# Tianxinhuang/RFNet

Hardware: AMD Instinct MI355X
Metric: point-pairs/sec Chamfer (BxNxM) (higher is better)
Workload: dtype f32; 1 GPU; Chamfer nn_distance fwd+bwd, B=32 per GPU, 2048 vs 16384 points (BASELINE.json configs[1]), randn seed 100; batch_per_gpu=32, n=2048, m=16384, step=rf_chamfer_step: one C-ABI call, caller-allocated outputs

## Files before the change

### rfnet_amd/csrc/nn_pruned.hip

```cpp
#include <stdlib.h>

#include <type_traits>

#include "common.hpp"
#include "nn_pruned.hpp"

namespace {

#ifndef RFP_NSH
#define RFP_NSH 4
#endif
#ifndef RFP_SPLIT_BELOW
#define RFP_SPLIT_BELOW 4096
#endif
#ifndef RFP_SORT_SPLIT
#define RFP_SORT_SPLIT 2
#endif
#ifndef RFP_SORT_SPLIT_ABOVE
#define RFP_SORT_SPLIT_ABOVE 8192
#endif
#ifndef RFP_WPE
#define RFP_WPE 7
#endif
#ifndef RFP_QSAMPLE
#define RFP_QSAMPLE 3
#endif
#ifndef RFP_STR_SMALL_N
#define RFP_STR_SMALL_N 4096
#endif
#ifndef RFP_CROWD_DIV
#define RFP_CROWD_DIV 4
#endif
#ifndef RFP_STR_LARGE_LEAF
#define RFP_STR_LARGE_LEAF 48
#endif
#ifndef RFP_STR_SMALL_LEAF
#define RFP_STR_SMALL_LEAF 32
#endif
#ifndef RFP_TILE16
#define RFP_TILE16 1
#endif
#ifndef RFP_KK1
#define RFP_KK1 1
#endif
#ifndef RFP_REKEY_BOX
#define RFP_REKEY_BOX 1
#endif
#ifndef RFP_REKEY_STATS
#define RFP_REKEY_STATS 0
#endif
constexpr int NSH = RFP_NSH;
constexpr int BS = 16;
constexpr int SBB = 4;
constexpr int SB = BS * SBB;
constexpr int KEYBITS = 15;
constexpr int NBINS = 1 << KEYBITS;
constexpr int STPB = 1024;
constexpr int RPT = 16;
constexpr int HB = 256;
static_assert(rfp::kMaxPoints / SB <= 1024, "superblock id must fit the key low 10 bits");
static_assert(!RFP_TILE16 || NSH == SBB, "the quad-per-query tiles need one wave per 16-record block of a group: RFP_NSH = 4");
constexpr unsigned IDMASK = 0x3FFu;
constexpr int B16F = SBB * 6;
constexpr int B64F = 8;

struct SortArgs {
    int b;
    int n[2], npad[2];
    const float *src[2];
    float *xyz[2];
    int *orig[2];
    float *box16[2];
    float *box64[2];
    int nsets;
    int split[2];
    int *pos0[2];
    int str_s[2];
    unsigned long long *dbg;
};

__device__ __forceinline__ int ragged_count(const int *__restrict__ len, int bi, int n) {
    if (!len) return n;
    const int v = len[bi];
    return v < 1 ? 1 : (v > n ? n : v);
}

__device__ __forceinline__ unsigned hilbert15(unsigned x, unsigned y, unsigned z) {
    unsigned X[3] = {x, y, z};
#pragma unroll
    for (unsigned Q = 16; Q > 1; Q >>= 1) {
        const unsigned P = Q - 1;
#pragma unroll
        for (int i = 0; i < 3; i++) {
            if (X[i] & Q) {
                X[0] ^= P;
            } else {
                const unsigned t = (X[0] ^ X[i]) & P;
                X[0] ^= t;
                X[i] ^= t;
            }
        }
    }
    X[1] ^= X[0];
    X[2] ^= X[1];
    unsigned t = 0;
#pragma unroll
    for (unsigned Q = 16; Q > 1; Q >>= 1)
        if (X[2] & Q) t ^= Q - 1;
    X[0] ^= t;
    X[1] ^= t;
    X[2] ^= t;
    unsigned key = 0;
#pragma unroll
    for (int bit = 0; bit < 5; bit++)
#pragma unroll
        for (int i = 0; i < 3; i++) key |= ((X[i] >> bit) & 1u) << (3 * bit + 2 - i);
    return key & (NBINS - 1);
}

__device__ __forceinline__ float axis_off(float lo, float scale) {
    return fmaf(-lo, scale, -0.5f);
}
__device__ __forceinline__ int axis_bin(float v, float off, float scale) {
    static_assert(HB == 256, "a bin is a byte");
    return (int)__builtin_amdgcn_cvt_pk_u8_f32(fmaf(v, scale, off), 0, 0u);
}
__device__ __forceinline__ float canon(float v) {
    asm volatile("v_max_f32 %0, %0, %0" : "+v"(v));
    return v;
}
__device__ __forceinline__ float bare_min(float a, float b) {
    float r;
    asm("v_min_f32 %0, %1, %2" : "=v"(r) : "v"(a), "v"(b));
    return r;
}
__device__ __forceinline__ float bare_max(float a, float b) {
    float r;
    asm("v_max_f32 %0, %1, %2" : "=v"(r) : "v"(a), "v"(b));
    return r;
}

__device__ __forceinline__ unsigned spread5(unsigned v) {
    v = (v | (v << 8)) & 0x100Fu;
    v = (v | (v << 4)) & 0x10C3u;
    v = (v | (v << 2)) & 0x1249u;
    return v;
}

__device__ __forceinline__ unsigned wave_incl_scan(unsigned v) {
    v += (unsigned)__builtin_amdgcn_update_dpp(0, (int)v, 0x111, 0xf, 0xf, false);
    v += (unsigned)__builtin_amdgcn_update_dpp(0, (int)v, 0x112, 0xf, 0xf, false);
    v += (unsigned)__builtin_amdgcn_update_dpp(0, (int)v, 0x114, 0xf, 0xf, false);
    v += (unsigned)__builtin_amdgcn_update_dpp(0, (int)v, 0x118, 0xf, 0xf, false);
    v += (unsigned)__builtin_amdgcn_update_dpp(0, (int)v, 0x142, 0xa, 0xf, false);
    v += (unsigned)__builtin_amdgcn_update_dpp(0, (int)v, 0x143, 0xc, 0xf, false);
    return v;
}

#define RFP_ROW(OP, N) asm volatile("s_nop 1\n\t" OP " %0, %0, %0 row_ror:" #N " row_mask:0xf bank_mask:0xf" : "+v"(v))
__device__ __forceinline__ float wave_min_f32(float v) {
    RFP_ROW("v_min_f32_dpp", 8);
    RFP_ROW("v_min_f32_dpp", 4);
    RFP_ROW("v_min_f32_dpp", 2);
    RFP_ROW("v_min_f32_dpp", 1);
    const float r0 = __int_as_float(__builtin_amdgcn_readlane(__float_as_int(v), 0));
    const float r1 = __int_as_float(__builtin_amdgcn_readlane(__float_as_int(v), 16));
    const float r2 = __int_as_float(__builtin_amdgcn_readlane(__float_as_int(v), 32));
    const float r3 = __int_as_float(__builtin_amdgcn_readlane(__float_as_int(v), 48));
    return fminf(fminf(r0, r1), fminf(r2, r3));
}
__device__ __forceinline__ float wave_max_f32(float v) {
    RFP_ROW("v_max_f32_dpp", 8);
    RFP_ROW("v_max_f32_dpp", 4);
    RFP_ROW("v_max_f32_dpp", 2);
    RFP_ROW("v_max_f32_dpp", 1);
    const float r0 = __int_as_float(__builtin_amdgcn_readlane(__float_as_int(v), 0));
    const float r1 = __int_as_float(__builtin_amdgcn_readlane(__float_as_int(v), 16));
    const float r2 = __int_as_float(__builtin_amdgcn_readlane(__float_as_int(v), 32));
    const float r3 = __int_as_float(__builtin_amdgcn_readlane(__float_as_int(v), 48));
    return fmaxf(fmaxf(r0, r1), fmaxf(r2, r3));
}
#undef RFP_ROW

__device__ __forceinline__ bool hist_is_dense(unsigned bin, bool act) {
    const unsigned long long todo = __builtin_amdgcn_ballot_w64(act);
    if (todo == 0ull) return false;
    const unsigned first = (unsigned)__builtin_amdgcn_readlane((int)bin, __builtin_ctzll(todo));
    return __builtin_popcountll(__builtin_amdgcn_ballot_w64(act && bin == first)) >= 8;
}

constexpr int HALF = 9216;

template <bool RAGGED, bool FLAG>
__global__ __launch_bounds__(STPB) void nnp_sort_reg_kernel(SortArgs a, const int *__restrict__ len0,
                                                            const int *__restrict__ len1) {
    struct Lds {
        unsigned ahist[3][HB];
        unsigned char slabmap[HB];
        unsigned short zmap[HB];
        unsigned char stripmap[16 * HB];
        float red[STPB / 64][6];
        unsigned wsum[STPB / 64];
        unsigned lowcnt[STPB / 64][3];
        float frame[6];
        unsigned ncrowded;
        unsigned badw[STPB / 64];
        __attribute__((aligned(16))) unsigned hist[HALF * 4];
    };
    __shared__ Lds lds;
    auto &hist = lds.hist;
    auto &ahist = lds.ahist;
    auto &slabmap = lds.slabmap;
    auto &zmap = lds.zmap;
    auto &stripmap = lds.stripmap;
    auto &red = lds.red;
    auto &wsum = lds.wsum;
    auto &lowcnt = lds.lowcnt;
    auto &frame = lds.frame;
    auto &ncrowded = lds.ncrowded;
    auto &badw = lds.badw;

    const int nwg = gridDim.x, q8 = nwg >> 3, r8 = nwg & 7, xcd = blockIdx.x & 7;
    const int logical = (xcd < r8 ? xcd * (q8 + 1) : r8 * (q8 + 1) + (xcd - r8) * q8) + (int)(blockIdx.x >> 3);
    if (threadIdx.x == 0) ncrowded = 0;
    const int wpb = a.split[0] + (a.nsets > 1 ? a.split[1] : 0);
    const int bi = logical / wpb;
    int rem = logical - bi * wpb;
    const int set = (a.nsets > 1 && rem >= a.split[0]) ? 1 : 0;
    if (set) rem -= a.split[0];
    const int H = a.split[set], half = rem;
    const int nfull = a.n[set], npad = a.npad[set];
    const float *__restrict__ src = a.src[set] + (size_t)bi * nfull * 3;
    const int n = RAGGED ? ragged_count(set ? len1 : len0, bi, nfull) : nfull;
    float *__restrict__ oxyz = a.xyz[set] + (size_t)bi * npad * 3;
    int *__restrict__ oorig = a.orig[set] + (size_t)bi * npad;
    const int tid = threadIdx.x, lane = tid & 63, wave = tid >> 6;
    int stamp_no = 16;
    auto stamp = [&]() {
        if (a.dbg && bi == a.b - 1 && set == a.nsets - 1 && half == H - 1 && tid == 0 && stamp_no < 32) a.dbg[stamp_no] = clock64();
        stamp_no++;
    };
    stamp();

    float px[RPT], py[RPT], pz[RPT];
    unsigned pk[RPT];
#pragma unroll
    for (int k = 0; k < RPT; k++) {
        const int i = tid + k * STPB;
        px[k] = py[k] = pz[k] = 0.f;
        if (i < n) {
            struct P3 {
                float x, y, z;
            };
            const P3 v = *(const P3 *)(src + (size_t)i * 3);
            px[k] = v.x;
            py[k] = v.y;
            pz[k] = v.z;
        }
    }
    {
        uint4 *h4 = (uint4 *)hist;
#pragma unroll
        for (int k = 0; k < NBINS / 4 / STPB; k++) h4[tid + k * STPB] = make_uint4(0, 0, 0, 0);
    }
    if (tid < 3 * HB) (&ahist[0][0])[tid] = 0;
    unsigned *yhist = hist + NBINS;
    for (int i = tid; i < 16 * HB; i += STPB) yhist[i] = 0;

    stamp();
    {
#pragma unroll
        for (int k = 0; k < RPT; k++) {
            px[k] = canon(px[k]);
            py[k] = canon(py[k]);
            pz[k] = canon(pz[k]);
        }
        float lo[3] = {INFINITY, INFINITY, INFINITY}, hi[3] = {-INFINITY, -INFINITY, -INFINITY};
#define RFP_BBOX_PASS(FILTER)                                                     \
    _Pragma("unroll") for (int k = 0; k < RPT; k++) {                             \
        if (tid + k * STPB < n) {                                                 \
            const float v[3] = {px[k], py[k], pz[k]};                             \
            _Pragma("unroll") for (int c = 0; c < 3; c++) {                       \
                if (!(FILTER) || isfinite(v[c])) {                                \
                    lo[c] = bare_min(lo[c], v[c]);                                \
                    hi[c] = bare_max(hi[c], v[c]);                                \
                }                                                                 \
            }                                                                     \
        }                                                                         \
    }                                                                             \
    _Pragma("unroll") for (int c = 0; c < 3; c++) {                               \
        lo[c] = wave_min_f32(lo[c]);                                              \
        hi[c] = wave_max_f32(hi[c]);                                              \
    }
        RFP_BBOX_PASS(false)
        if (!(isfinite(lo[0]) && isfinite(lo[1]) && isfinite(lo[2]) && isfinite(hi[0]) && isfinite(hi[1]) && isfinite(hi[2]))) {
#pragma unroll
            for (int c = 0; c < 3; c++) {
                lo[c] = INFINITY;
                hi[c] = -INFINITY;
            }
            RFP_BBOX_PASS(true)
        }
#undef RFP_BBOX_PASS
        if (lane == 0) {
#pragma unroll
            for (int c = 0; c < 3; c++) {
                red[wave][c] = lo[c];
                red[wave][3 + c] = hi[c];
            }
        }
        if (FLAG) {
            float nf = 0.f;
#pragma unroll
            for (int k = 0; k < RPT; k++) nf = fmaf(pz[k], 0.f, fmaf(py[k], 0.f, fmaf(px[k], 0.f, nf)));
            const unsigned long long bad_lanes = __ballot(nf != nf);
            if (lane == 0) badw[wave] = bad_lanes != 0ull ? 1u : 0u;
        }
    }
    __syncthreads();
    if (tid < 3) {
        float l = INFINITY, h = -INFINITY;
        for (int w = 0; w < STPB / 64; w++) {
            l = bare_min(l, red[w][tid]);
            h = bare_max(h, red[w][3 + tid]);
        }
        const float ext = h - l;
        const bool ok = isfinite(ext) && ext > 0.f;
        frame[tid] = ok ? l : 0.f;
        frame[3 + tid] = ok ? (float)HB / ext : 0.f;
    }
    __syncthreads();
    const float fs[3] = {frame[3], frame[4], frame[5]};
    const float fl[3] = {axis_off(frame[0], fs[0]), axis_off(frame[1], fs[1]), axis_off(frame[2], fs[2])};

    stamp();
    bool dense;
    {
        const int w3 = wave & RFP_QSAMPLE;
        const float x0 = w3 == 0 ? px[0] : (w3 == 3 ? px[1] : (w3 == 2 ? px[2] : px[3]));
        const int k0 = (4 - w3) & 3;
        dense = RFP_QSAMPLE == 3 && hist_is_dense((unsigned)axis_bin(x0, fl[0], fs[0]), tid + k0 * STPB < n);
    }
    const bool feeds = !dense || (lane & 3) == 0;
    if (dense && lane == 0) atomicAdd(&ncrowded, 1u);
#pragma unroll
    for (int k = 0; k < RPT; k++) {
        if (((k + wave) & RFP_QSAMPLE) != 0) continue;
        if (feeds && tid + k * STPB < n) {
            atomicAdd(&ahist[0][axis_bin(px[k], fl[0], fs[0])], 1u);
            atomicAdd(&ahist[2][axis_bin(pz[k], fl[2], fs[2])], 1u);
        }
        __builtin_amdgcn_sched_barrier(0);
    }
    __syncthreads();
    const int SS = a.str_s[set];
    if (wave == 0 || wave == 2) {
        unsigned c4[4], sm = 0;
#pragma unroll
        for (int k = 0; k < 4; k++) {
            c4[k] = ahist[wave][lane * 4 + k];
            sm += c4[k];
        }
        const unsigned incl = wave_incl_scan(sm);
        const unsigned total = max((unsigned)__builtin_amdgcn_readlane((int)incl, 63), 1u);
        unsigned run = incl - sm;
        const float per = (wave == 0 ? (float)SS : 512.f) / (float)total;
#pragma unroll
        for (int k = 0; k < 4; k++) {
            const unsigned q = (unsigned)((float)run * per);
            if (wave == 0) {
                slabmap[lane * 4 + k] = (unsigned char)(q > (unsigned)SS - 1u ? (unsigned)SS - 1u : q);
            } else {
                zmap[lane * 4 + k] = (unsigned short)(q > 511u ? 511u : q);
            }
            run += c4[k];
        }
    }
    __syncthreads();
#pragma unroll
    for (int k = 0; k < RPT; k++) {
        if (((k + wave) & RFP_QSAMPLE) != 0) continue;
        if (feeds && tid + k * STPB < n)
            atomicAdd(&yhist[(int)slabmap[axis_bin(px[k], fl[0], fs[0])] * HB + axis_bin(py[k], fl[1], fs[1])], 1u);
    }
    __syncthreads();
    if (wave < SS) {
        unsigned c4[4], sm = 0;
#pragma unroll
        for (int k = 0; k < 4; k++) {
            c4[k] = yhist[wave * HB + lane * 4 + k];
            sm += c4[k];
        }
        const unsigned incl = wave_incl_scan(sm);
        const unsigned total = max((unsigned)__builtin_amdgcn_readlane((int)incl, 63), 1u);
        unsigned run = incl - sm;
        const float per = (float)SS / (float)total;
#pragma unroll
        for (int k = 0; k < 4; k++) {
            unsigned st = (unsigned)((float)run * per);
            st = st > (unsigned)SS - 1u ? (unsigned)SS - 1u : st;
            stripmap[wave * HB + lane * 4 + k] = (unsigned char)((wave & 1) ? (unsigned)SS - 1u - st : st);
            run += c4[k];
        }
    }
    __syncthreads();
    const int ncol = SS * SS;
    auto col_start = [&](int q) { return (q * ncol + H - 1) / H; };
    const int cs1 = H > 1 ? col_start(1) : 0x7FFFFFFF;
#if RFP_SORT_SPLIT > 2
    const int cs2 = H > 2 ? col_start(2) : 0x7FFFFFFF, cs3 = H > 3 ? col_start(3) : 0x7FFFFFFF;
#endif
    const unsigned kbase = (unsigned)col_start(half) << 9;
    const int nb_local = (col_start(half + 1) - col_start(half)) << 9;

    stamp();
    unsigned below[3] = {0u, 0u, 0u};
    const unsigned dkeep = dense ? ~15u : ~0u, dlane = dense ? (unsigned)(lane & 15) : 0u;
#pragma unroll
    for (int k = 0; k < RPT; k++) {
        const bool valid = tid + k * STPB < n;
        const int xb = axis_bin(px[k], fl[0], fs[0]), yb = axis_bin(py[k], fl[1], fs[1]);
        const int slab = slabmap[xb];
        const int col = (int)__umul24(slab, SS) + (int)stripmap[slab * HB + yb];
#if RFP_SORT_SPLIT > 2
        int slice = col >= cs1;
        if (H > 2) slice += (col >= cs2) + (col >= cs3);
        const bool own = valid && slice == half;
#pragma unroll
        for (int q = 0; q < 3; q++) below[q] += (unsigned)__builtin_popcountll(__builtin_amdgcn_ballot_w64(valid && slice == q));
#else
        const bool own = valid && (col >= cs1) == (half != 0);
#endif
        unsigned zq = zmap[axis_bin(pz[k], fl[2], fs[2])];
        zq = (zq & dkeep) | dlane;
        const unsigned key = ((unsigned)col << 9) | ((col & 1) ? 511u - zq : zq);
        pk[k] = own ? key - kbase : 0xFFFFFFFFu;
        if (own) atomicAdd(&hist[pk[k]], 1u);
    }
#if RFP_SORT_SPLIT <= 2
    if (half == 1) {
#pragma unroll
        for (int k = 0; k < RPT; k++) {
            const int nv = n - (__builtin_amdgcn_readfirstlane(wave) * 64 + k * STPB);
            below[0] += (unsigned)(nv < 0 ? 0 : (nv > 64 ? 64 : nv)) - (unsigned)__builtin_popcountll(__builtin_amdgcn_ballot_w64(pk[k] != 0xFFFFFFFFu));
        }
    }
#endif
    if (H > 1 && lane == 0) {
#pragma unroll
        for (int q = 0; q < 3; q++) lowcnt[wave][q] = q < half ? below[q] : 0u;
    }
    __syncthreads();

    stamp();
    int cown = 0;
    {
        constexpr int STEPS = NBINS / (STPB / 64) / 256;
        const int steps = min(STEPS, (nb_local + 4095) / 4096);
        uint4 *h4 = (uint4 *)hist + (size_t)wave * steps * 64;
        uint4 v[STEPS];
        unsigned tot = 0;
#pragma unroll
        for (int it = 0; it < STEPS; it++) {
            v[it] = it < steps ? h4[it * 64 + lane] : make_uint4(0, 0, 0, 0);
            tot += v[it].x + v[it].y + v[it].z + v[it].w;
        }
        tot = wave_incl_scan(tot);
        if (lane == 63) wsum[wave] = tot;
        __syncthreads();
        const unsigned wtot = lane < STPB / 64 ? wsum[lane] : 0u;
        const unsigned wincl = wave_incl_scan(wtot);
        unsigned carry = (unsigned)__builtin_amdgcn_readlane((int)(wincl - wtot), __builtin_amdgcn_readfirstlane(wave));
        cown = __builtin_amdgcn_readlane((int)wincl, STPB / 64 - 1);
#pragma unroll
        for (int it = 0; it < STEPS; it++) {
            if (it < steps) {
                const unsigned sm = v[it].x + v[it].y + v[it].z + v[it].w;
                const unsigned incl = wave_incl_scan(sm);
                uint4 out;
                out.x = carry + incl - sm;
                out.y = out.x + v[it].x;
                out.z = out.y + v[it].y;
                out.w = out.z + v[it].z;
                h4[it * 64 + lane] = out;
                carry += (unsigned)__builtin_amdgcn_readlane((int)incl, 63);
            }
        }
    }
    __syncthreads();

    stamp();
#pragma unroll
    for (int k = 0; k < RPT; k++)
        if (pk[k] != 0xFFFFFFFFu) pk[k] = atomicAdd(&hist[pk[k]], 1u);
    __syncthreads();

    stamp();
    float4 *stg = (float4 *)hist;
    float *__restrict__ b16 = a.box16[set] + (size_t)bi * (npad / SB) * B16F;
    float *__restrict__ b64 = a.box64[set] + (size_t)bi * (npad / SB) * B64F;
    int base = 0;
    for (int q = 0; q < half; q++) {
        unsigned c = 0;
        for (int w = 0; w < STPB / 64; w++) c += lowcnt[w][q];
        base += ((int)c + SB - 1) / SB * SB;
    }
    const int seglen = ((cown + SB - 1) / SB) * SB;
    if (half == H - 1) {
        const int t0 = base + seglen;
        for (int j = t0 * 3 + tid; j < npad * 3; j += STPB) oxyz[j] = INFINITY;
        for (int j = t0 + tid; j < npad; j += STPB) oorig[j] = -1;
        for (int j = (t0 / SB) * B16F + tid; j < (npad / SB) * B16F; j += STPB) b16[j] = ((j % 6) < 3) ? INFINITY : -INFINITY;
        for (int j = (t0 / SB) * B64F + tid; j < (npad / SB) * B64F; j += STPB) {
            const int c = j % B64F;
            b64[j] = c < 3 ? INFINITY : (c >= 4 && c < 7 ? -INFINITY : 0.f);
        }
    }
    if (tid == 0 && pk[0] != 0xFFFFFFFFu) a.pos0[set][bi] = base + (int)pk[0];
    if (tid == 0 && half == 0) {
        a.pos0[set][a.b + bi] = ncrowded * RFP_CROWD_DIV > STPB / 64 ? 1 : 0;
        if (FLAG) {
            unsigned nbad = 0;
            for (int w = 0; w < STPB / 64; w++) nbad |= badw[w];
            a.pos0[set][2 * a.b + bi] = nbad != 0u ? 1 : 0;
        }
    }
    for (int h0 = 0; h0 < seglen; h0 += HALF) {
        const int cnt = min(HALF, seglen - h0);
#pragma unroll
        for (int k = 0; k < RPT; k++) {
            const int i = tid + k * STPB;
            const int p = (int)pk[k] - h0;
            if (pk[k] != 0xFFFFFFFFu && p >= 0 && p < HALF) stg[p] = make_float4(px[k], py[k], pz[k], __int_as_float(i));
        }
        for (int p = cown - h0 + tid; p < cnt; p += STPB)
            if (p >= 0) stg[p] = make_float4(INFINITY, INFINITY, INFINITY, __int_as_float(-1));
        __syncthreads();
        stamp();
#pragma unroll 1
        for (int t2 = tid; t2 < cnt / BS * 2; t2 += STPB) {
            const int blk = t2 >> 1, hf = t2 & 1;
            float l[3] = {INFINITY, INFINITY, INFINITY}, hh[3] = {-INFINITY, -INFINITY, -INFINITY};
#pragma unroll 4
            for (int u = 0; u < BS / 2; u++) {
                const int r = blk * BS + hf * (BS / 2) + ((u + blk + 4 * hf) & (BS / 2 - 1));
                const float4 v = stg[r];
                if (h0 + r < cown) {
                    l[0] = bare_min(l[0], v.x); hh[0] = bare_max(hh[0], v.x);
                    l[1] = bare_min(l[1], v.y); hh[1] = bare_max(hh[1], v.y);
                    l[2] = bare_min(l[2], v.z); hh[2] = bare_max(hh[2], v.z);
                }
            }
#pragma unroll
            for (int c = 0; c < 3; c++) {
                l[c] = bare_min(l[c], __shfl_xor(l[c], 1, 64));
                hh[c] = bare_max(hh[c], __shfl_xor(hh[c], 1, 64));
            }
            const int gblk = (base + h0) / BS + blk;
            if (hf == 0) {
                float *o = b16 + (size_t)(gblk >> 2) * B16F + (gblk & 3) * 6;
#pragma unroll
                for (int c = 0; c < 3; c++) {
                    o[c] = l[c];
                    o[3 + c] = hh[c];
                }
            }
#pragma unroll
            for (int x = 2; x <= 4; x <<= 1) {
#pragma unroll
                for (int c = 0; c < 3; c++) {
                    l[c] = bare_min(l[c], __shfl_xor(l[c], x, 64));
                    hh[c] = bare_max(hh[c], __shfl_xor(hh[c], x, 64));
                }
            }
            if ((gblk & 3) == 0 && hf == 0) {
                float *o64 = b64 + (size_t)(gblk >> 2) * B64F;
#pragma unroll
                for (int c = 0; c < 3; c++) {
                    o64[c] = l[c];
                    o64[4 + c] = hh[c];
                }
                o64[3] = o64[7] = 0.f;
            }
        }
        stamp();
        {
            struct P3 {
                float x, y, z;
            };
            for (int j = tid; j < cnt; j += STPB) {
                const float4 v = stg[j];
                *(P3 *)(oxyz + (size_t)(base + h0 + j) * 3) = P3{v.x, v.y, v.z};
                oorig[base + h0 + j] = __float_as_int(v.w);
            }
        }
        __syncthreads();
        stamp();
    }
}

template <bool REG, bool RAGGED>
__global__ __launch_bounds__(STPB) void nnp_sort_kernel(SortArgs a, const int *__restrict__ len0,
                                                        const int *__restrict__ len1) {
    __shared__ __attribute__((aligned(16))) unsigned hist[NBINS];
    __shared__ unsigned ahist[3][HB];
    __shared__ unsigned char cellmap[3][HB];
    __shared__ float red[STPB / 64][6];
    __shared__ unsigned wsum[STPB / 64];
    __shared__ float frame[6];
    __shared__ unsigned nbad;

    const int nwg = gridDim.x, q8 = nwg >> 3, r8 = nwg & 7, xcd = blockIdx.x & 7;
    const int logical = (xcd < r8 ? xcd * (q8 + 1) : r8 * (q8 + 1) + (xcd - r8) * q8) + (int)(blockIdx.x >> 3);
    const int bi = logical / a.nsets, set = logical - bi * a.nsets;
    if (threadIdx.x == 0) nbad = 0;
    const int nfull = a.n[set], npad = a.npad[set];
    const float *__restrict__ src = a.src[set] + (size_t)bi * nfull * 3;
    const int n = RAGGED ? ragged_count(set ? len1 : len0, bi, nfull) : nfull;
    float *__restrict__ oxyz = a.xyz[set] + (size_t)bi * npad * 3;
    int *__restrict__ oorig = a.orig[set] + (size_t)bi * npad;
    const int tid = threadIdx.x, lane = tid & 63, wave = tid >> 6;

    float px[REG ? RPT : 1], py[REG ? RPT : 1], pz[REG ? RPT : 1];
    unsigned pkey[REG ? RPT : 1];
    if constexpr (REG) {
#pragma unroll
        for (int k = 0; k < RPT; k++) {
            const int i = tid + k * STPB;
            px[k] = py[k] = pz[k] = 0.f;
            if (i < n) {
                px[k] = src[(size_t)i * 3 + 0];
                py[k] = src[(size_t)i * 3 + 1];
                pz[k] = src[(size_t)i * 3 + 2];
            }
        }
    }
    auto for_points = [&](auto f) {
        if constexpr (REG) {
#pragma unroll
            for (int k = 0; k < RPT; k++) {
                const int i = tid + k * STPB;
                if (i < n) f(k, i, px[k], py[k], pz[k]);
            }
        } else {
            for (int i = tid; i < n; i += STPB) f(0, i, src[(size_t)i * 3 + 0], src[(size_t)i * 3 + 1], src[(size_t)i * 3 + 2]);
        }
    };

    for (int i = tid; i < NBINS; i += STPB) hist[i] = 0;
    if (tid < 3 * HB) (&ahist[0][0])[tid] = 0;

    float lo[3] = {INFINITY, INFINITY, INFINITY}, hi[3] = {-INFINITY, -INFINITY, -INFINITY};
    bool bad = false;
    __syncthreads();
    for_points([&](int, int, float x, float y, float z) {
        const float v[3] = {x, y, z};
#pragma unroll
        for (int c = 0; c < 3; c++) {
            if (isfinite(v[c])) {
                lo[c] = fminf(lo[c], v[c]);
                hi[c] = fmaxf(hi[c], v[c]);
            } else {
                bad = true;
            }
        }
    });
    if (__ballot(bad) != 0ull && lane == 0) nbad = 1u;
#pragma unroll
    for (int o = 32; o > 0; o >>= 1) {
#pragma unroll
        for (int c = 0; c < 3; c++) {
            lo[c] = fminf(lo[c], __shfl_xor(lo[c], o, 64));
            hi[c] = fmaxf(hi[c], __shfl_xor(hi[c], o, 64));
        }
    }
    if (lane == 0) {
#pragma unroll
        for (int c = 0; c < 3; c++) {
            red[wave][c] = lo[c];
            red[wave][3 + c] = hi[c];
        }
    }
    __syncthreads();
    if (tid < 3) {
        float l = INFINITY, h = -INFINITY;
        for (int w = 0; w < STPB / 64; w++) {
            l = fminf(l, red[w][tid]);
            h = fmaxf(h, red[w][3 + tid]);
        }
        const float ext = h - l;
        const bool ok = isfinite(ext) && ext > 0.f;
        frame[tid] = ok ? l : 0.f;
        frame[3 + tid] = ok ? (float)HB / ext : 0.f;
    }
    __syncthreads();
    const float fs[3] = {frame[3], frame[4], frame[5]};
    const float fl[3] = {axis_off(frame[0], fs[0]), axis_off(frame[1], fs[1]), axis_off(frame[2], fs[2])};

    for_points([&](int, int i, float x, float y, float z) {
        if ((((unsigned)i >> 10) + (unsigned)i) & 3u) return;
        atomicAdd(&ahist[0][axis_bin(x, fl[0], fs[0])], 1u);
        atomicAdd(&ahist[1][axis_bin(y, fl[1], fs[1])], 1u);
        atomicAdd(&ahist[2][axis_bin(z, fl[2], fs[2])], 1u);
    });
    __syncthreads();
    if (wave < 3) {
        unsigned c4[4], s = 0;
#pragma unroll
        for (int k = 0; k < 4; k++) {
            c4[k] = ahist[wave][lane * 4 + k];
            s += c4[k];
        }
        unsigned incl = s;
#pragma unroll
        for (int o = 1; o < 64; o <<= 1) {
            const unsigned v = __shfl_up(incl, o, 64);
            if (lane >= o) incl += v;
        }
        const unsigned total = max(__shfl(incl, 63, 64), 1u);
        unsigned run = incl - s;
#pragma unroll
        for (int k = 0; k < 4; k++) {
            const unsigned cell = (run * 32u) / total;
            cellmap[wave][lane * 4 + k] = (unsigned char)(cell > 31u ? 31u : cell);
            run += c4[k];
        }
    }
    __syncthreads();

    auto key_of = [&](float x, float y, float z) {
        const unsigned cx = cellmap[0][axis_bin(x, fl[0], fs[0])];
        const unsigned cy = cellmap[1][axis_bin(y, fl[1], fs[1])];
        const unsigned cz = cellmap[2][axis_bin(z, fl[2], fs[2])];
        return hilbert15(cx, cy, cz);
    };

    for_points([&](int k, int, float x, float y, float z) {
        const unsigned key = key_of(x, y, z);
        if constexpr (REG) pkey[k] = key;
        atomicAdd(&hist[key], 1u);
    });
    __syncthreads();

    {
        constexpr int STEPS = NBINS / STPB / 4 * 0 + (NBINS / (STPB / 64) / 256);
        uint4 *h4 = (uint4 *)hist + (size_t)wave * (NBINS / (STPB / 64) / 4);
        unsigned tot = 0;
#pragma unroll
        for (int it = 0; it < STEPS; it++) {
            const uint4 v = h4[it * 64 + lane];
            tot += v.x + v.y + v.z + v.w;
        }
#pragma unroll
        for (int o = 32; o > 0; o >>= 1) tot += __shfl_xor(tot, o, 64);
        if (lane == 0) wsum[wave] = tot;
        __syncthreads();
        unsigned carry = 0;
        for (int w = 0; w < wave; w++) carry += wsum[w];
#pragma unroll
        for (int it = 0; it < STEPS; it++) {
            const uint4 v = h4[it * 64 + lane];
            const unsigned sm = v.x + v.y + v.z + v.w;
            unsigned incl = sm;
#pragma unroll
            for (int o = 1; o < 64; o <<= 1) {
                const unsigned t = __shfl_up(incl, o, 64);
                if (lane >= o) incl += t;
            }
            uint4 out;
            out.x = carry + incl - sm;
            out.y = out.x + v.x;
            out.z = out.y + v.y;
            out.w = out.z + v.z;
            h4[it * 64 + lane] = out;
            carry += __shfl(incl, 63, 64);
        }
    }
    __syncthreads();

    for_points([&](int k, int i, float x, float y, float z) {
        unsigned key;
        if constexpr (REG) key = pkey[k];
        else key = key_of(x, y, z);
        const unsigned pos = atomicAdd(&hist[key], 1u);
        if (i == 0) {
            a.pos0[set][bi] = (int)pos;
            a.pos0[set][a.b + bi] = 0;
            a.pos0[set][2 * a.b + bi] = nbad != 0u ? 1 : 0;
        }
        oxyz[(size_t)pos * 3 + 0] = x;
        oxyz[(size_t)pos * 3 + 1] = y;
        oxyz[(size_t)pos * 3 + 2] = z;
        oorig[pos] = i;
    });
    for (int i = n + tid; i < npad; i += STPB) {
        oxyz[(size_t)i * 3 + 0] = INFINITY;
        oxyz[(size_t)i * 3 + 1] = INFINITY;
        oxyz[(size_t)i * 3 + 2] = INFINITY;
        oorig[i] = -1;
    }
    __syncthreads();

    float *__restrict__ b16 = a.box16[set] + (size_t)bi * (npad / SB) * B16F;
    float *__restrict__ b64 = a.box64[set] + (size_t)bi * (npad / SB) * B64F;
    for (int blk = tid; blk < npad / BS; blk += STPB) {
        float l[3] = {INFINITY, INFINITY, INFINITY}, h[3] = {-INFINITY, -INFINITY, -INFINITY};
        const float *p = oxyz + (size_t)blk * BS * 3;
        const int *po = oorig + (size_t)blk * BS;
        for (int u = 0; u < BS; u++) {
            if (po[u] >= 0) {
#pragma unroll
                for (int c = 0; c < 3; c++) {
                    l[c] = fminf(l[c], p[u * 3 + c]);
                    h[c] = fmaxf(h[c], p[u * 3 + c]);
                }
            }
        }
        float *o = b16 + (size_t)(blk >> 2) * B16F + (blk & 3) * 6;
#pragma unroll
        for (int c = 0; c < 3; c++) {
            o[c] = l[c];
            o[3 + c] = h[c];
        }
#pragma unroll
        for (int x = 1; x <= 2; x <<= 1) {
#pragma unroll
            for (int c = 0; c < 3; c++) {
                l[c] = fminf(l[c], __shfl_xor(l[c], x, 64));
                h[c] = fmaxf(h[c], __shfl_xor(h[c], x, 64));
            }
        }
        if ((blk & 3) == 0) {
            float *o64 = b64 + (size_t)(blk >> 2) * B64F;
#pragma unroll
            for (int c = 0; c < 3; c++) {
                o64[c] = l[c];
                o64[4 + c] = h[c];
            }
            o64[3] = o64[7] = 0.f;
        }
    }
}


struct SweepArgs {
    int b;
    int n[2], npad[2];
    int groups[2];
    int nw[2];
    int wg0, wg1;
    int kstride;
};

struct GradEmit {
    const float *gd[2];
    char *base;
    int qbucket[2];
};
struct EmitView {
    int4 *rec;
    unsigned long long *mask;
};
__host__ __device__ inline size_t emit_align(size_t v) { return (v + 255) / 256 * 256; }
__host__ __device__ inline size_t emit_set_bytes(int b, int npad) {
    return emit_align((size_t)b * npad * sizeof(int4)) + emit_align((size_t)b * (npad / 64) * sizeof(unsigned long long));
}
__host__ __device__ inline EmitView emit_layout(char *base, int b, int npad0, int npad1, int set) {
    char *p = base + (set ? emit_set_bytes(b, npad0) : 0);
    const int npad = set ? npad1 : npad0;
    EmitView v;
    v.rec = (int4 *)p;
    p += emit_align((size_t)b * npad * sizeof(int4));
    v.mask = (unsigned long long *)p;
    return v;
}

__device__ __forceinline__ float min3_acc(float acc, float a, float b) {
    asm("v_min3_f32 %0, %0, %1, %2" : "+v"(acc) : "v"(a), "v"(b));
    return acc;
}

#define RFP_DPP(OP, N) asm volatile("s_nop 1\n\t" OP " %0, %0, %0 row_ror:" #N " row_mask:0xf bank_mask:0xf" : "+v"(v))
__device__ __forceinline__ unsigned wave_min_u32(unsigned v) {
    RFP_DPP("v_min_u32_dpp", 8);
    RFP_DPP("v_min_u32_dpp", 4);
    RFP_DPP("v_min_u32_dpp", 2);
    RFP_DPP("v_min_u32_dpp", 1);
    const unsigned r0 = __builtin_amdgcn_readlane(v, 0), r1 = __builtin_amdgcn_readlane(v, 16);
    const unsigned r2 = __builtin_amdgcn_readlane(v, 32), r3 = __builtin_amdgcn_readlane(v, 48);
    return min(min(r0, r1), min(r2, r3));
}
__device__ __forceinline__ float wave_max_nonneg(float f) {
    unsigned v = f < 0.f ? 0u : __float_as_uint(f);
    RFP_DPP("v_max_u32_dpp", 8);
    RFP_DPP("v_max_u32_dpp", 4);
    RFP_DPP("v_max_u32_dpp", 2);
// ... 1298 lines not shown
```

Measured before the change: 15040 billion pairs/s.

## Reuse first-pass histogram ranks, batch block scans, and interleave box/copy roles

The first histogram pass now keeps each point's atomicAdd return value, a within-bin rank, packed into the upper bits of its local key. The scatter pass then reads the scanned bin offset and adds that rank, so the second round of LDS atomics is no longer needed. The exclusive scan over histogram steps is split into independent groups of four per-step wave scans, so they no longer form one serial dependency chain. In the staging loop, waves alternate by parity between computing the box bounds and copying sorted points out, so the two phases overlap instead of running back to back. This adds packing assumptions, guarded by static_asserts, and leaves uneven work between waves.

```diff
diff --git a/rfnet_amd/csrc/nn_pruned.hip b/rfnet_amd/csrc/nn_pruned.hip
--- a/rfnet_amd/csrc/nn_pruned.hip
+++ b/rfnet_amd/csrc/nn_pruned.hip
@@ -21,6 +21,15 @@
 #endif
 #ifndef RFP_WPE
 #define RFP_WPE 7
+#endif
+#ifndef RFP_SORT_ROLES
+#define RFP_SORT_ROLES 1
+#endif
+#ifndef RFP_SORT_RANK1
+#define RFP_SORT_RANK1 1
+#endif
+#ifndef RFP_SORT_SCAN4
+#define RFP_SORT_SCAN4 1
 #endif
 #ifndef RFP_QSAMPLE
 #define RFP_QSAMPLE 3
@@ -416,6 +425,9 @@
     stamp();
     unsigned below[3] = {0u, 0u, 0u};
     const unsigned dkeep = dense ? ~15u : ~0u, dlane = dense ? (unsigned)(lane & 15) : 0u;
+#if RFP_SORT_RANK1
+    unsigned rk[RPT];
+#endif
 #pragma unroll
     for (int k = 0; k < RPT; k++) {
         const bool valid = tid + k * STPB < n;
@@ -435,8 +447,19 @@
         zq = (zq & dkeep) | dlane;
         const unsigned key = ((unsigned)col << 9) | ((col & 1) ? 511u - zq : zq);
         pk[k] = own ? key - kbase : 0xFFFFFFFFu;
+#if RFP_SORT_RANK1
+        static_assert(RPT * STPB <= (1 << (31 - KEYBITS)), "a rank and a local key share one register");
+        if (k > 0) asm volatile("v_lshl_or_b32 %0, %1, 15, %0" : "+v"(pk[k - 1]) : "v"(rk[k - 1]));
+        asm("" : "=v"(rk[k]));
+        if (own) rk[k] = atomicAdd(&hist[pk[k]], 1u);
+#else
         if (own) atomicAdd(&hist[pk[k]], 1u);
-    }
+#endif
+    }
+#if RFP_SORT_RANK1
+    pk[RPT - 1] |= rk[RPT - 1] << KEYBITS;
+    static_assert(KEYBITS == 15, "the shift of the merge in the keys loop");
+#endif
 #if RFP_SORT_SPLIT <= 2
     if (half == 1) {
 #pragma unroll
@@ -472,6 +495,33 @@
         const unsigned wincl = wave_incl_scan(wtot);
         unsigned carry = (unsigned)__builtin_amdgcn_readlane((int)(wincl - wtot), __builtin_amdgcn_readfirstlane(wave));
         cown = __builtin_amdgcn_readlane((int)wincl, STPB / 64 - 1);
+#if RFP_SORT_SCAN4
+        unsigned stot[STEPS];
+#pragma unroll
+        for (int i0 = 0; i0 < STEPS; i0 += 4) {
+            if (i0 == 0 || steps > i0) {
+#pragma unroll
+                for (int it = i0; it < i0 + 4; it++) {
+                    const unsigned sm = v[it].x + v[it].y + v[it].z + v[it].w;
+                    const unsigned incl = wave_incl_scan(sm);
+                    v[it].w = incl - sm;
+                    stot[it] = (unsigned)__builtin_amdgcn_readlane((int)incl, 63);
+                }
+            }
+        }
+#pragma unroll
+        for (int it = 0; it < STEPS; it++) {
+            if (it < steps) {
+                uint4 out;
+                out.x = carry + v[it].w;
+                out.y = out.x + v[it].x;
+                out.z = out.y + v[it].y;
+                out.w = out.z + v[it].z;
+                h4[it * 64 + lane] = out;
+                carry += stot[it];
+            }
+        }
+#else
 #pragma unroll
         for (int it = 0; it < STEPS; it++) {
             if (it < steps) {
@@ -486,13 +536,20 @@
                 carry += (unsigned)__builtin_amdgcn_readlane((int)incl, 63);
             }
         }
+#endif
     }
     __syncthreads();
 
     stamp();
+#if RFP_SORT_RANK1
+#pragma unroll
+    for (int k = 0; k < RPT; k++)
+        if (pk[k] != 0xFFFFFFFFu) pk[k] = hist[pk[k] & (unsigned)(NBINS - 1)] + (pk[k] >> KEYBITS);
+#else
 #pragma unroll
     for (int k = 0; k < RPT; k++)
         if (pk[k] != 0xFFFFFFFFu) pk[k] = atomicAdd(&hist[pk[k]], 1u);
+#endif
     __syncthreads();
 
     stamp();
@@ -537,61 +594,70 @@
             if (p >= 0) stg[p] = make_float4(INFINITY, INFINITY, INFINITY, __int_as_float(-1));
         __syncthreads();
         stamp();
+#if RFP_SORT_ROLES == 0
+        const int role0 = 0;
+#pragma unroll
+#else
+        const int role0 = (__builtin_amdgcn_readfirstlane(wave) >> (RFP_SORT_ROLES == 1 ? 0 : RFP_SORT_ROLES == 2 ? 3 : 2)) & 1;
 #pragma unroll 1
-        for (int t2 = tid; t2 < cnt / BS * 2; t2 += STPB) {
-            const int blk = t2 >> 1, hf = t2 & 1;
-            float l[3] = {INFINITY, INFINITY, INFINITY}, hh[3] = {-INFINITY, -INFINITY, -INFINITY};
+#endif
+        for (int role = 0; role < 2; role++) {
+            if (role == role0) {
+#pragma unroll 1
+                for (int t2 = tid; t2 < cnt / BS * 2; t2 += STPB) {
+                    const int blk = t2 >> 1, hf = t2 & 1;
+                    float l[3] = {INFINITY, INFINITY, INFINITY}, hh[3] = {-INFINITY, -INFINITY, -INFINITY};
 #pragma unroll 4
-            for (int u = 0; u < BS / 2; u++) {
-                const int r = blk * BS + hf * (BS / 2) + ((u + blk + 4 * hf) & (BS / 2 - 1));
-                const float4 v = stg[r];
-                if (h0 + r < cown) {
-                    l[0] = bare_min(l[0], v.x); hh[0] = bare_max(hh[0], v.x);
-                    l[1] = bare_min(l[1], v.y); hh[1] = bare_max(hh[1], v.y);
-                    l[2] = bare_min(l[2], v.z); hh[2] = bare_max(hh[2], v.z);
+                    for (int u = 0; u < BS / 2; u++) {
+                        const int r = blk * BS + hf * (BS / 2) + ((u + blk + 4 * hf) & (BS / 2 - 1));
+                        const float4 v = stg[r];
+                        if (h0 + r < cown) {
+                            l[0] = bare_min(l[0], v.x); hh[0] = bare_max(hh[0], v.x);
+                            l[1] = bare_min(l[1], v.y); hh[1] = bare_max(hh[1], v.y);
+                            l[2] = bare_min(l[2], v.z); hh[2] = bare_max(hh[2], v.z);
+                        }
+                    }
+#pragma unroll
+                    for (int c = 0; c < 3; c++) {
+                        l[c] = bare_min(l[c], __shfl_xor(l[c], 1, 64));
+                        hh[c] = bare_max(hh[c], __shfl_xor(hh[c], 1, 64));
+                    }
+                    const int gblk = (base + h0) / BS + blk;
+                    if (hf == 0) {
+                        float *o = b16 + (size_t)(gblk >> 2) * B16F + (gblk & 3) * 6;
+#pragma unroll
+                        for (int c = 0; c < 3; c++) {
+                            o[c] = l[c];
+                            o[3 + c] = hh[c];
+                        }
+                    }
+#pragma unroll
+                    for (int x = 2; x <= 4; x <<= 1) {
+#pragma unroll
+                        for (int c = 0; c < 3; c++) {
+                            l[c] = bare_min(l[c], __shfl_xor(l[c], x, 64));
+                            hh[c] = bare_max(hh[c], __shfl_xor(hh[c], x, 64));
+                        }
+                    }
+                    if ((gblk & 3) == 0 && hf == 0) {
+                        float *o64 = b64 + (size_t)(gblk >> 2) * B64F;
+#pragma unroll
+                        for (int c = 0; c < 3; c++) {
+                            o64[c] = l[c];
+                            o64[4 + c] = hh[c];
+                        }
+                        o64[3] = o64[7] = 0.f;
+                    }
                 }
-            }
-#pragma unroll
-            for (int c = 0; c < 3; c++) {
-                l[c] = bare_min(l[c], __shfl_xor(l[c], 1, 64));
-                hh[c] = bare_max(hh[c], __shfl_xor(hh[c], 1, 64));
-            }
-            const int gblk = (base + h0) / BS + blk;
-            if (hf == 0) {
-                float *o = b16 + (size_t)(gblk >> 2) * B16F + (gblk & 3) * 6;
-#pragma unroll
-                for (int c = 0; c < 3; c++) {
-                    o[c] = l[c];
-                    o[3 + c] = hh[c];
+            } else {
+                struct P3 {
+                    float x, y, z;
+                };
+                for (int j = tid; j < cnt; j += STPB) {
+                    const float4 v = stg[j];
+                    *(P3 *)(oxyz + (size_t)(base + h0 + j) * 3) = P3{v.x, v.y, v.z};
+                    oorig[base + h0 + j] = __float_as_int(v.w);
                 }
-            }
-#pragma unroll
-            for (int x = 2; x <= 4; x <<= 1) {
-#pragma unroll
-                for (int c = 0; c < 3; c++) {
-                    l[c] = bare_min(l[c], __shfl_xor(l[c], x, 64));
-                    hh[c] = bare_max(hh[c], __shfl_xor(hh[c], x, 64));
-                }
-            }
-            if ((gblk & 3) == 0 && hf == 0) {
-                float *o64 = b64 + (size_t)(gblk >> 2) * B64F;
-#pragma unroll
-                for (int c = 0; c < 3; c++) {
-                    o64[c] = l[c];
-                    o64[4 + c] = hh[c];
-                }
-                o64[3] = o64[7] = 0.f;
-            }
-        }
-        stamp();
-        {
-            struct P3 {
-                float x, y, z;
-            };
-            for (int j = tid; j < cnt; j += STPB) {
-                const float4 v = stg[j];
-                *(P3 *)(oxyz + (size_t)(base + h0 + j) * 3) = P3{v.x, v.y, v.z};
-                oorig[base + h0 + j] = __float_as_int(v.w);
             }
         }
         __syncthreads();
```

After: 15030 billion pairs/s (median of 2 runs). No clear change (-0.0%).
